# harskish/ganspace

Measured on NVIDIA H100. Metric: latent samples/sec into PCA (StyleGAN2-ffhq W, N=1e6), higher is better.
Workload: dtype f32

## Files before the change

### ganspace_b200/csrc/mapping_tc.cu

```cuda
#include "tc_common.cuh"
#include <stdlib.h>

namespace gsb {

constexpr int TC_BLOCK_M = 128;
constexpr int TC_BLOCK_N = 128;
constexpr int TC_BLOCK_K = 64;
constexpr int TC_STAGES = 3;
constexpr int TC_FRAG_ROWS = 64;
constexpr uint32_t TC_A_BYTES = TC_BLOCK_M * TC_BLOCK_K * 2;
constexpr uint32_t TC_W_BYTES = TC_BLOCK_N * TC_BLOCK_K * 2;
constexpr uint32_t TC_STAGE_BYTES = 2 * TC_A_BYTES + 2 * TC_W_BYTES;
constexpr uint32_t TC_BOX_BYTES = TC_FRAG_ROWS * 128;
constexpr uint32_t TC_STAGING_BYTES = 2 * 2 * TC_BOX_BYTES;
constexpr int TC_THREADS = tc::CONSUMER_THREADS + 128;
constexpr uint32_t TC_SMEM_BYTES = TC_STAGES * TC_STAGE_BYTES + TC_STAGING_BYTES + 64  + 1024 ;
static_assert(TC_SMEM_BYTES <= 232448, "mapping_layer_tc_kernel: shared memory exceeds the H100's 227 KB per block");

struct TcParams {
    const float *bias;
    __half *out_hi;
    __half *out_lo;
    float *out_f32;
    unsigned *overflow;
    const float *inv_wscale;
    int M, N_total, K;
    int mode;
    int dbg;
};

__global__ void __launch_bounds__(TC_THREADS, 1)
mapping_layer_tc_kernel(const __grid_constant__ CUtensorMap tm_a_hi, const __grid_constant__ CUtensorMap tm_a_lo,
                        const __grid_constant__ CUtensorMap tm_w_hi, const __grid_constant__ CUtensorMap tm_w_lo,
                        const __grid_constant__ CUtensorMap tm_o0, const __grid_constant__ CUtensorMap tm_o1,
                        const TcParams p) {
    using namespace tc;
    extern __shared__ uint8_t smem_raw[];
    uint8_t *smem = reinterpret_cast<uint8_t *>((reinterpret_cast<uintptr_t>(smem_raw) + 1023) & ~(uintptr_t)1023);
    uint8_t *staging = smem + TC_STAGES * TC_STAGE_BYTES;
    uint64_t *bars = reinterpret_cast<uint64_t *>(staging + TC_STAGING_BYTES);
    uint64_t *full_bar = bars;
    uint64_t *empty_bar = bars + TC_STAGES;
    uint64_t *turn_bar = bars + 2 * TC_STAGES;

    const int warp = threadIdx.x >> 5, lane = threadIdx.x & 31;
    const int num_m_tiles = (p.M + TC_BLOCK_M - 1) / TC_BLOCK_M;
    const int num_n_tiles = (p.N_total + TC_BLOCK_N - 1) / TC_BLOCK_N;
    const int num_k_blocks = (p.K + TC_BLOCK_K - 1) / TC_BLOCK_K;
    const int num_units = num_m_tiles * num_n_tiles;

    if (threadIdx.x == 0) {
        for (int s = 0; s < TC_STAGES; ++s) { mbar_init(&full_bar[s], 1); mbar_init(&empty_bar[s], 4); }
        mbar_init(&turn_bar[0], 4); mbar_init(&turn_bar[1], 4);
        mbar_fence_init();
    }
    if (warp == PRODUCER_WARP && lane == 0) {
        tma_prefetch_desc(&tm_a_hi); tma_prefetch_desc(&tm_a_lo);
        tma_prefetch_desc(&tm_w_hi); tma_prefetch_desc(&tm_w_lo);
        tma_prefetch_desc(&tm_o0); tma_prefetch_desc(&tm_o1);
    }
    __syncthreads();

    if (warp >= PRODUCER_WARP) {
        asm volatile("setmaxnreg.dec.sync.aligned.u32 40;");
        if (warp == PRODUCER_WARP && lane == 0) {
            int stage = 0; uint32_t phase = 0;
            for (int u = blockIdx.x; u < num_units; u += gridDim.x) {
                const int m0 = (u / num_n_tiles) * TC_BLOCK_M, n0 = (u % num_n_tiles) * TC_BLOCK_N;
                for (int kb = 0; kb < num_k_blocks; ++kb) {
                    mbar_wait(&empty_bar[stage], phase ^ 1);
                    uint8_t *st = smem + stage * TC_STAGE_BYTES;
                    mbar_arrive_expect_tx(&full_bar[stage], ((p.dbg & 4) ? 0u : 2 * TC_A_BYTES) + ((p.dbg & 2) ? 0u : 2 * TC_W_BYTES));
                    if (!(p.dbg & 4)) {
                        tma_load_2d(&tm_a_hi, &full_bar[stage], st, kb * TC_BLOCK_K, m0);
                        tma_load_2d(&tm_a_lo, &full_bar[stage], st + TC_A_BYTES, kb * TC_BLOCK_K, m0);
                    }
                    if (!(p.dbg & 2)) {
                        tma_load_2d(&tm_w_hi, &full_bar[stage], st + 2 * TC_A_BYTES, kb * TC_BLOCK_K, n0);
                        tma_load_2d(&tm_w_lo, &full_bar[stage], st + 2 * TC_A_BYTES + TC_W_BYTES, kb * TC_BLOCK_K, n0);
                    }
                    if (++stage == TC_STAGES) { stage = 0; phase ^= 1; }
                }
            }
        }
    } else {
        asm volatile("setmaxnreg.inc.sync.aligned.u32 232;");
        const int wg = warp >> 2;
        const int rr0 = (warp & 3) * 16 + (lane >> 2);
        const int q2 = 2 * (lane & 3);
        const bool has_bias = (p.mode != 1);
        const float slope = (p.mode == 0) ? 0.2f : 1.0f, gain = (p.mode == 0) ? 1.41421356237309515f : 1.0f;
        const float inv_wscale = __ldg(p.inv_wscale);
        uint8_t *stg = staging + wg * (2 * TC_BOX_BYTES);
        const bool storer = ((threadIdx.x & 127) == 0);
        const bool to_f32 = (p.out_f32 != nullptr);
        bool ovf = false;
        float acc0[64], acc1[64];
#pragma unroll
        for (int j = 0; j < 64; ++j) { acc0[j] = 0.f; acc1[j] = 0.f; }

        auto store_chunk = [&](const float (&acc)[64], const int ib, const int mrow, const int n0, const int c0) {
            if (storer) asm volatile("cp.async.bulk.wait_group.read 0;" ::: "memory");
            asm volatile("bar.sync %0, 128;" ::"r"(1 + wg) : "memory");
#pragma unroll
            for (int g = 0; g < 8; ++g) {
                const int col = n0 + c0 + 8 * g + q2;
                float2 b = make_float2(0.f, 0.f);
                if (has_bias && col < p.N_total) b = __ldg(reinterpret_cast<const float2 *>(p.bias + col));
#pragma unroll
                for (int h = 0; h < 2; ++h) {
                    const int rr = rr0 + 8 * h;
                    float f[2];
#pragma unroll
                    for (int e = 0; e < 2; ++e) {
                        float x = __fmul_rn(acc[ib + 4 * g + 2 * h + e], inv_wscale) + (e ? b.y : b.x);
                        x = (x >= 0.f) ? x : __fmul_rn(x, slope);
                        f[e] = __fmul_rn(gain, x);
                    }
                    uint8_t *row = stg + rr * 128;
                    const uint32_t sw = (uint32_t)(rr & 7);
                    if (to_f32) {
                        const int cb = (8 * g + q2) & 31;
                        *reinterpret_cast<float2 *>(row + (g >> 2) * TC_BOX_BYTES + ((((uint32_t)cb >> 2) ^ sw) << 4) + (cb & 3) * 4) =
                            make_float2(f[0], f[1]);
                    } else {
                        uint32_t hi, lo;
                        split2(f[0], f[1], hi, lo);
                        ovf |= (fabsf(f[0]) > 60000.f) | (fabsf(f[1]) > 60000.f);
                        *reinterpret_cast<uint32_t *>(row + (((uint32_t)g ^ sw) << 4) + 2 * q2) = hi;
                        *reinterpret_cast<uint32_t *>(row + TC_BOX_BYTES + (((uint32_t)g ^ sw) << 4) + 2 * q2) = lo;
                    }
                }
            }
            asm volatile("fence.proxy.async.shared::cta;" ::: "memory");
            asm volatile("bar.sync %0, 128;" ::"r"(1 + wg) : "memory");
            if (storer && !(p.dbg & 1) && n0 + c0 < p.N_total) {
                if (to_f32) {
                    tma_store_2d(&tm_o0, stg, n0 + c0, mrow);
                    if (n0 + c0 + 32 < p.N_total) tma_store_2d(&tm_o0, stg + TC_BOX_BYTES, n0 + c0 + 32, mrow);
                } else {
                    tma_store_2d(&tm_o0, stg, n0 + c0, mrow);
                    tma_store_2d(&tm_o1, stg + TC_BOX_BYTES, n0 + c0, mrow);
                }
                asm volatile("cp.async.bulk.commit_group;" ::: "memory");
            }
        };

        for (int i = wg;; i += 2) {
            const int u = blockIdx.x + i * gridDim.x;
            if (u >= num_units) break;
            const int m0 = (u / num_n_tiles) * TC_BLOCK_M, n0 = (u % num_n_tiles) * TC_BLOCK_N;
            const int g0 = i * num_k_blocks;
            int stage = g0 % TC_STAGES, prev = stage;
            uint32_t phase = (uint32_t)(g0 / TC_STAGES) & 1;
            if (i > 0) mbar_wait(&turn_bar[wg], (uint32_t)((i - 1) >> 1) & 1);
            for (int kb = 0; kb < num_k_blocks; ++kb) {
                mbar_wait(&full_bar[stage], phase);
                if (!(p.dbg & 8)) {
                    const uint32_t st = smem_u32(smem + stage * TC_STAGE_BYTES);
                    const uint32_t sw = st + 2 * TC_A_BYTES;
                    const uint64_t d_wh = sw128_kmajor_desc(sw), d_wl = sw128_kmajor_desc(sw + TC_W_BYTES);
                    wgmma_fence();
                    split_kblock_m64n128(acc0, sw128_kmajor_desc(st), sw128_kmajor_desc(st + TC_A_BYTES), d_wh, d_wl, kb > 0);
                    split_kblock_m64n128(acc1, sw128_kmajor_desc(st + TC_A_BYTES / 2),
                                         sw128_kmajor_desc(st + TC_A_BYTES + TC_A_BYTES / 2), d_wh, d_wl, kb > 0);
                    wgmma_commit();
                }
                wgmma_wait_1();
                if (kb > 0 && lane == 0) mbar_arrive(&empty_bar[prev]);
                if (kb == num_k_blocks - 1 && lane == 0) mbar_arrive(&turn_bar[wg ^ 1]);
                prev = stage;
                if (++stage == TC_STAGES) { stage = 0; phase ^= 1; }
            }
            wgmma_wait_all();
            if (lane == 0) mbar_arrive(&empty_bar[prev]);
            store_chunk(acc0, 0, m0, n0, 0);
            store_chunk(acc0, 32, m0, n0, 64);
            store_chunk(acc1, 0, m0 + TC_FRAG_ROWS, n0, 0);
            store_chunk(acc1, 32, m0 + TC_FRAG_ROWS, n0, 64);
        }
        if (ovf) atomicOr(p.overflow, 1u);
        if (storer) asm volatile("cp.async.bulk.wait_group 0;" ::: "memory");
    }
}

__global__ void pixelnorm_split_kernel(const float *__restrict__ x, __half *__restrict__ hi, __half *__restrict__ lo,
                                       int64_t n, int dim, int do_norm, unsigned *overflow) {
    int64_t row = blockIdx.x * (int64_t)(blockDim.x >> 5) + (threadIdx.x >> 5);
    if (row >= n) return;
    const int lane = threadIdx.x & 31;
    const float4 *xr = reinterpret_cast<const float4 *>(x + row * dim);
    float r = 1.f;
    if (do_norm) {
        float s = 0.f;
        for (int i = lane; i < dim / 4; i += 32) {
            float4 v = xr[i];
            s += v.x * v.x + v.y * v.y + v.z * v.z + v.w * v.w;
        }
        s = warp_sum(s);
        r = 1.0f / sqrtf(s / (float)dim + 1e-8f);
    }
    bool ovf = false;
    for (int i = lane; i < dim / 4; i += 32) {
        float4 v = xr[i];
        const float f[4] = {v.x * r, v.y * r, v.z * r, v.w * r};
        uint2 ph, pl;
        ovf |= tc::split4(f, ph, pl);
        reinterpret_cast<uint2 *>(hi + row * dim)[i] = ph;
        reinterpret_cast<uint2 *>(lo + row * dim)[i] = pl;
    }
    if (ovf) atomicOr(overflow, 1u);
}

__global__ void pick_wscale_kernel(const float *__restrict__ absmax, float *__restrict__ wscale,
                                   float *__restrict__ inv_wscale) {
    float m = *absmax;
    if (!(m > 0.f)) m = 1.f;
    int e = 0;
    frexpf(m, &e);
    const int s = 14 - e;
    *wscale = ldexpf(1.f, s);
    *inv_wscale = ldexpf(1.f, -s);
}

__global__ void weight_split_kernel(const float *__restrict__ pw, int64_t count, const float *__restrict__ wscale_p,
                                    __half *__restrict__ hi, __half *__restrict__ lo) {
    const float wscale = *wscale_p;
    for (int64_t i = blockIdx.x * (int64_t)blockDim.x + threadIdx.x; i < count; i += (int64_t)gridDim.x * blockDim.x) {
        tc::split1(pw[i] * wscale, hi[i], lo[i]);
    }
}

__global__ void absmax_kernel(const float *__restrict__ x, int64_t count, float *__restrict__ out) {
    float m = 0.f;
    for (int64_t i = blockIdx.x * (int64_t)blockDim.x + threadIdx.x; i < count; i += (int64_t)gridDim.x * blockDim.x)
        m = fmaxf(m, fabsf(x[i]));
    for (int o = 16; o > 0; o >>= 1) m = fmaxf(m, __shfl_xor_sync(0xffffffffu, m, o));
    if ((threadIdx.x & 31) == 0) atomicMax(reinterpret_cast<int *>(out), __float_as_int(m));
}

static int make_tmap(CUtensorMap *map, const void *base, uint64_t rows, uint64_t cols, uint32_t box_rows,
                     CUtensorMapDataType type = CU_TENSOR_MAP_DATA_TYPE_FLOAT16) {
    const uint32_t esize = (type == CU_TENSOR_MAP_DATA_TYPE_FLOAT32) ? 4 : 2;
    const uint64_t dims[2] = {cols, rows};
    const uint64_t strides[1] = {cols * esize};
    const uint32_t box[2] = {128 / esize, box_rows};
    return tc_make_tmap(map, type, base, 2, dims, strides, box);
}

size_t mapping_tc_packed_bytes(int n_layers, int dim) {
    return align_up((size_t)n_layers * dim * dim * 2, 256) * 2 + align_up((size_t)3 * n_layers * sizeof(float), 256) + 256;
}

struct TcPackView {
    __half *w_hi, *w_lo;
    float *inv_wscale, *wscale, *absmax;
    unsigned *overflow;
};
static TcPackView tc_pack_view(void *base, int n_layers, int dim) {
    TcPackView v;
    char *p = reinterpret_cast<char *>(base);
    size_t wb = align_up((size_t)n_layers * dim * dim * 2, 256);
    v.w_hi = reinterpret_cast<__half *>(p);
    v.w_lo = reinterpret_cast<__half *>(p + wb);
    v.inv_wscale = reinterpret_cast<float *>(p + 2 * wb);
    v.wscale = v.inv_wscale + n_layers;
    v.absmax = v.wscale + n_layers;
    v.overflow = reinterpret_cast<unsigned *>(p + 2 * wb + align_up((size_t)3 * n_layers * sizeof(float), 256));
    return v;
}

int mapping_tc_pack(const float *pw, int n_layers, int dim, void *tc_base, cudaStream_t st) {
    TcPackView v = tc_pack_view(tc_base, n_layers, dim);
    GSB_CHECK_CUDA(cudaMemsetAsync(v.inv_wscale, 0, (size_t)3 * n_layers * sizeof(float), st));
    GSB_CHECK_CUDA(cudaMemsetAsync(v.overflow, 0, sizeof(unsigned), st));
    const int64_t per = (int64_t)dim * dim;
    for (int l = 0; l < n_layers; ++l) {
        absmax_kernel<<<64, 256, 0, st>>>(pw + l * per, per, v.absmax + l);
        GSB_CHECK_LAUNCH();
        pick_wscale_kernel<<<1, 1, 0, st>>>(v.absmax + l, v.wscale + l, v.inv_wscale + l);
        GSB_CHECK_LAUNCH();
        weight_split_kernel<<<256, 256, 0, st>>>(pw + l * per, per, v.wscale + l, v.w_hi + l * per, v.w_lo + l * per);
        GSB_CHECK_LAUNCH();
    }
    return GSB_OK;
}

static int tc_ensure_attr() {
    static bool attr_set = false;
    if (!attr_set) {
        GSB_CHECK_CUDA(cudaFuncSetAttribute(mapping_layer_tc_kernel, cudaFuncAttributeMaxDynamicSharedMemorySize, (int)TC_SMEM_BYTES));
        attr_set = true;
    }
    return GSB_OK;
}

static int tc_launch_layer(const CUtensorMap &tm_ah, const CUtensorMap &tm_al, const CUtensorMap &tm_wh, const CUtensorMap &tm_wl,
                           TcParams p, int leave_free_sms, cudaStream_t st) {
    CUtensorMap tm_o0, tm_o1;
    if (p.out_f32) {
        if (int r = make_tmap(&tm_o0, p.out_f32, (uint64_t)p.M, (uint64_t)p.N_total, TC_FRAG_ROWS,
                              CU_TENSOR_MAP_DATA_TYPE_FLOAT32))
            return r;
        tm_o1 = tm_o0;
    } else {
        if (int r = make_tmap(&tm_o0, p.out_hi, (uint64_t)p.M, (uint64_t)p.N_total, TC_FRAG_ROWS)) return r;
        if (int r = make_tmap(&tm_o1, p.out_lo, (uint64_t)p.M, (uint64_t)p.N_total, TC_FRAG_ROWS)) return r;
    }
    const int m_tiles = (p.M + TC_BLOCK_M - 1) / TC_BLOCK_M, n_tiles = (p.N_total + TC_BLOCK_N - 1) / TC_BLOCK_N;
    int avail = num_sms() - leave_free_sms;
    if (avail < 16) avail = 16;
    if (avail > num_sms()) avail = num_sms();
    {
        static int dbg = -1;
        if (dbg < 0) { const char *e = getenv("GANSPACE_B200_MAPPING_DBG"); dbg = e ? atoi(e) : 0; }
        p.dbg = dbg;
    }
    const int64_t units = (int64_t)m_tiles * n_tiles;
    const int grid = units < avail ? (int)units : avail;
    mapping_layer_tc_kernel<<<grid, TC_THREADS, TC_SMEM_BYTES, st>>>(tm_ah, tm_al, tm_wh, tm_wl, tm_o0, tm_o1, p);
    GSB_CHECK_LAUNCH();
    return GSB_OK;
}

int tc_gemm_plain(const __half *a_hi, const __half *a_lo, int64_t M, int K, const __half *w_hi, const __half *w_lo, int N,
                  const float *inv_wscale, float *out, unsigned *overflow, int leave_free_sms, cudaStream_t st) {
    GSB_CHECK_ARG(N % 32 == 0 && N >= 32 && K % 8 == 0 && K >= 8 && M > 0 && M < (1ll << 31),
                  "tc_gemm_plain: need N%%32==0, K%%8==0 (M=%lld N=%d K=%d)", (long long)M, N, K);
    if (int r = tc_ensure_attr()) return r;
    CUtensorMap tm_ah, tm_al, tm_wh, tm_wl;
    if (int r = make_tmap(&tm_ah, a_hi, (uint64_t)M, (uint64_t)K, TC_BLOCK_M)) return r;
    if (int r = make_tmap(&tm_al, a_lo, (uint64_t)M, (uint64_t)K, TC_BLOCK_M)) return r;
    if (int r = make_tmap(&tm_wh, w_hi, (uint64_t)N, (uint64_t)K, TC_BLOCK_N)) return r;
    if (int r = make_tmap(&tm_wl, w_lo, (uint64_t)N, (uint64_t)K, TC_BLOCK_N)) return r;
    TcParams p;
    p.bias = nullptr; p.out_hi = nullptr; p.out_lo = nullptr; p.out_f32 = out; p.overflow = overflow;
    p.inv_wscale = inv_wscale; p.M = (int)M; p.N_total = N; p.K = K; p.mode = 1;
    return tc_launch_layer(tm_ah, tm_al, tm_wh, tm_wl, p, leave_free_sms, st);
}

size_t tc_linear_workspace_bytes(int64_t n, int N, int K) {
    return 2 * align_up((size_t)n * K * 2, 256) + 2 * align_up((size_t)N * K * 2, 256) + 512;
}

int tc_linear(const float *x, const float *w, const float *bias, float *y, int64_t n, int N, int K, bool lrelu, void *ws,
              cudaStream_t st) {
    GSB_CHECK_ARG(N % 256 == 0 && K % TC_BLOCK_K == 0 && n > 0 && n < (1ll << 31) && bias, "tc_linear: need N%%256==0, K%%64==0, bias");
    if (int r = tc_ensure_attr()) return r;
    char *p0 = reinterpret_cast<char *>(ws);
    const size_t xb = align_up((size_t)n * K * 2, 256), wb = align_up((size_t)N * K * 2, 256);
    __half *x_hi = (__half *)p0, *x_lo = (__half *)(p0 + xb), *w_hi = (__half *)(p0 + 2 * xb), *w_lo = (__half *)(p0 + 2 * xb + wb);
    float *scal = (float *)(p0 + 2 * xb + 2 * wb);
    unsigned *overflow = (unsigned *)(p0 + 2 * xb + 2 * wb + 256);
    GSB_CHECK_CUDA(cudaMemsetAsync(scal, 0, 512, st));
    absmax_kernel<<<256, 256, 0, st>>>(w, (int64_t)N * K, scal + 2);
    GSB_CHECK_LAUNCH();
    pick_wscale_kernel<<<1, 1, 0, st>>>(scal + 2, scal + 1, scal);
    GSB_CHECK_LAUNCH();
    weight_split_kernel<<<1024, 256, 0, st>>>(w, (int64_t)N * K, scal + 1, w_hi, w_lo);
    GSB_CHECK_LAUNCH();
    pixelnorm_split_kernel<<<(unsigned)((n + 7) / 8), 256, 0, st>>>(x, x_hi, x_lo, n, K, 0, overflow);
    GSB_CHECK_LAUNCH();
    CUtensorMap tm_ah, tm_al, tm_wh, tm_wl;
    if (int r = make_tmap(&tm_ah, x_hi, (uint64_t)n, (uint64_t)K, TC_BLOCK_M)) return r;
    if (int r = make_tmap(&tm_al, x_lo, (uint64_t)n, (uint64_t)K, TC_BLOCK_M)) return r;
    if (int r = make_tmap(&tm_wh, w_hi, (uint64_t)N, (uint64_t)K, TC_BLOCK_N)) return r;
    if (int r = make_tmap(&tm_wl, w_lo, (uint64_t)N, (uint64_t)K, TC_BLOCK_N)) return r;
    TcParams p;
    p.bias = bias; p.out_hi = nullptr; p.out_lo = nullptr; p.out_f32 = y; p.overflow = overflow;
    p.inv_wscale = scal; p.M = (int)n; p.N_total = N; p.K = K; p.mode = lrelu ? 0 : 2;
    return tc_launch_layer(tm_ah, tm_al, tm_wh, tm_wl, p, 0, st);
}

int mapping_forward_tc(const float *pb, void *tc_base, int n_layers, int dim,
                       const float *d_z, float *d_w, int64_t n, bool pixelnorm, void *ws, int leave_free_sms,
                       cudaStream_t st) {
    GSB_CHECK_ARG(dim % 256 == 0 && dim % TC_BLOCK_K == 0, "mapping_forward_tc: dim must be a multiple of 256");
    GSB_CHECK_ARG(n < (1ll << 31), "mapping_forward_tc: too many rows");
    TcPackView v = tc_pack_view(tc_base, n_layers, dim);
    const size_t buf = align_up((size_t)n * dim * 2, 256);
    __half *a_hi[2] = {reinterpret_cast<__half *>(ws), reinterpret_cast<__half *>((char *)ws + 2 * buf)};
    __half *a_lo[2] = {reinterpret_cast<__half *>((char *)ws + buf), reinterpret_cast<__half *>((char *)ws + 3 * buf)};

    if (int r = tc_ensure_attr()) return r;
    pixelnorm_split_kernel<<<(unsigned)((n + 7) / 8), 256, 0, st>>>(d_z, a_hi[0], a_lo[0], n, dim, pixelnorm ? 1 : 0,
                                                                  v.overflow);
    GSB_CHECK_LAUNCH();
    const int64_t per = (int64_t)dim * dim;
    for (int l = 0; l < n_layers; ++l) {
        const int src = l & 1, dst = src ^ 1;
        CUtensorMap tm_ah, tm_al, tm_wh, tm_wl;
        if (int r = make_tmap(&tm_ah, a_hi[src], (uint64_t)n, dim, TC_BLOCK_M)) return r;
        if (int r = make_tmap(&tm_al, a_lo[src], (uint64_t)n, dim, TC_BLOCK_M)) return r;
        if (int r = make_tmap(&tm_wh, v.w_hi + l * per, dim, dim, TC_BLOCK_N)) return r;
        if (int r = make_tmap(&tm_wl, v.w_lo + l * per, dim, dim, TC_BLOCK_N)) return r;
        TcParams p;
        p.bias = pb + (int64_t)l * dim;
        const bool last = (l == n_layers - 1);
        p.out_hi = last ? nullptr : a_hi[dst];
        p.out_lo = last ? nullptr : a_lo[dst];
        p.out_f32 = last ? d_w : nullptr;
        p.overflow = v.overflow;
        p.inv_wscale = v.inv_wscale + l;
        p.M = (int)n; p.N_total = dim; p.K = dim; p.mode = 0;
        if (int r = tc_launch_layer(tm_ah, tm_al, tm_wh, tm_wl, p, leave_free_sms, st)) return r;
    }
    return GSB_OK;
}

size_t mapping_tc_workspace_bytes(int64_t n, int dim) { return 4 * align_up((size_t)n * dim * 2, 256); }

unsigned *mapping_tc_overflow_flag(void *tc_base, int n_layers, int dim) {
    return tc_pack_view(tc_base, n_layers, dim).overflow;
}

}
```

### ganspace_b200/csrc/synthesis.cu

```cuda
#include "tc_common.cuh"
#include <math.h>

namespace gsb {

constexpr int SY_MAX_LAYERS = 24;
constexpr int SY_CHUNK_ROWS = 2048;

struct SynthLayerView {
    __half *w_hi, *w_lo;
    float *scal;
    float *wsq;
    float *modw;
    float *modb;
    float *actb;
    float *noise;
};
struct SynthView {
    float *const_nhwc;
    float *zeros;
    unsigned *overflow;
    SynthLayerView L[SY_MAX_LAYERS];
    size_t bytes;
};
static int res_out_of(const gsb_styled_conv &l) { return l.upsample ? 2 * l.res_in : l.res_in; }
// ... 163 lines not shown
    for (int k = 0; k < 4; ++k) f[k] = sqrt2 * ((f[k] >= 0.f) ? f[k] : 0.2f * f[k]);
    if (e.rgb_w) {
        const float4 sr = *reinterpret_cast<const float4 *>(e.rgb_s + b * c + 4 * q);
        const float g[4] = {f[0] * sr.x, f[1] * sr.y, f[2] * sr.z, f[3] * sr.w};
        float r[3];
#pragma unroll
        for (int o = 0; o < 3; ++o) {
            const float4 wv = *reinterpret_cast<const float4 *>(e.rgb_w + (int64_t)o * c + 4 * q);
            r[o] = e.rgb_scale * (g[0] * wv.x + g[1] * wv.y + g[2] * wv.z + g[3] * wv.w);
        }
        const int cq = c >> 2, span = cq < 32 ? cq : 32;
        for (int off = span >> 1; off > 0; off >>= 1) {
#pragma unroll
            for (int o = 0; o < 3; ++o) r[o] += __shfl_xor_sync(0xffffffffu, r[o], off);
        }
        float *dst = e.rgb_out + (b * hw + pix) * 3;
        if (cq <= 32) {
            if ((q & (span - 1)) == 0) { dst[0] += r[0]; dst[1] += r[1]; dst[2] += r[2]; }
        } else {
            __shared__ float rgb_red[8][3];
            const int wib = threadIdx.x >> 5, wpp = cq >> 5;
            if ((threadIdx.x & 31) == 0) { rgb_red[wib][0] = r[0]; rgb_red[wib][1] = r[1]; rgb_red[wib][2] = r[2]; }
            __syncthreads();
            if ((threadIdx.x & 31) == 0 && (wib % wpp) == 0) {
                float t0 = 0.f, t1 = 0.f, t2 = 0.f;
                for (int k = 0; k < wpp; ++k) { t0 += rgb_red[wib + k][0]; t1 += rgb_red[wib + k][1]; t2 += rgb_red[wib + k][2]; }
                dst[0] += t0; dst[1] += t1; dst[2] += t2;
            }
            __syncthreads();
        }
    }
    if (e.s_next) {
        const float4 sn = *reinterpret_cast<const float4 *>(e.s_next + b * c + 4 * q);
        f[0] *= sn.x; f[1] *= sn.y; f[2] *= sn.z; f[3] *= sn.w;
        bool ovf = false;
        store_split4(f, e.out_hi, e.out_lo, (b * hw + pix) * (int64_t)c + 4 * q, ovf);
        if (ovf) atomicOr(e.overflow, 1u);
    } else if (e.out_f32) {
        *reinterpret_cast<float4 *>(e.out_f32 + b * e.ld + (int64_t)pix * c + 4 * q) = make_float4(f[0], f[1], f[2], f[3]);
    }
}

__global__ void sy_rgb_init_kernel(const float *__restrict__ bias, const float *__restrict__ prev, int64_t n, int R, float *__restrict__ rgb) {
    const int64_t idx = blockIdx.x * (int64_t)blockDim.x + threadIdx.x;
    if (idx >= n * R * R) return;
    const int x = (int)(idx % R), y = (int)((idx / R) % R);
    const int64_t b = idx / ((int64_t)R * R);
    float acc[3] = {bias[0], bias[1], bias[2]};
    if (prev) {
        const int Rp = R >> 1;
        const float k1[4] = {1.f, 3.f, 3.f, 1.f};
#pragma unroll
        for (int i = 0; i < 4; ++i) {
            const int u = y + i - 2;
            if (u < 0 || (u & 1) || (u >> 1) >= Rp) continue;
#pragma unroll
            for (int j = 0; j < 4; ++j) {
                const int v = x + j - 2;
                if (v < 0 || (v & 1) || (v >> 1) >= Rp) continue;
                const float kw = k1[i] * k1[j] * 0.0625f;
                const float *pp = prev + ((b * Rp + (u >> 1)) * Rp + (v >> 1)) * 3;
                acc[0] = fmaf(kw, pp[0], acc[0]); acc[1] = fmaf(kw, pp[1], acc[1]); acc[2] = fmaf(kw, pp[2], acc[2]);
            }
        }
    }
    float *o = rgb + idx * 3;
    o[0] = acc[0]; o[1] = acc[1]; o[2] = acc[2];
}

__global__ void __launch_bounds__(256)
sy_conv_gather_kernel(const float *__restrict__ Y, int64_t nb, int H, int W, int c, EpiParams e) {
    const int cq = c >> 2;
    const int64_t idx = blockIdx.x * (int64_t)blockDim.x + threadIdx.x;
    if (idx >= nb * H * W * cq) return;
    const int q = (int)(idx % cq);
    const int64_t pixg = idx / cq;
    const int x = (int)(pixg % W), y = (int)((pixg / W) % H);
    const int64_t b = pixg / ((int64_t)W * H);
    float4 acc = make_float4(0.f, 0.f, 0.f, 0.f);
#pragma unroll
    for (int ky = 0; ky < 3; ++ky) {
        const int yy = y + ky - 1;
        if (yy < 0 || yy >= H) continue;
#pragma unroll
        for (int kx = 0; kx < 3; ++kx) {
            const int xx = x + kx - 1;
            if (xx < 0 || xx >= W) continue;
            const float4 v = *reinterpret_cast<const float4 *>(Y + ((b * H + yy) * W + xx) * (int64_t)(9 * c) + (ky * 3 + kx) * c + 4 * q);
            acc.x += v.x; acc.y += v.y; acc.z += v.z; acc.w += v.w;
        }
    }
    sy_epilogue(e, acc, b, y * W + x, H * W, c, q);
}

__global__ void __launch_bounds__(256)
sy_upconv_scatter_kernel(const float *__restrict__ Y, int64_t nb, int H, int W, int c, float *__restrict__ T) {
    const int cq = c >> 2, TH = 2 * H + 1, TW = 2 * W + 1;
    const int64_t idx = blockIdx.x * (int64_t)blockDim.x + threadIdx.x;
    if (idx >= nb * TH * TW * cq) return;
    const int q = (int)(idx % cq);
    const int64_t pixg = idx / cq;
    const int v = (int)(pixg % TW), u = (int)((pixg / TW) % TH);
    const int64_t b = pixg / ((int64_t)TW * TH);
    float4 acc = make_float4(0.f, 0.f, 0.f, 0.f);
#pragma unroll
    for (int ky = 0; ky < 3; ++ky) {
        const int t = u - ky;
        if (t < 0 || (t & 1) || (t >> 1) >= H) continue;
        const int yy = t >> 1;
#pragma unroll
        for (int kx = 0; kx < 3; ++kx) {
            const int s = v - kx;
            if (s < 0 || (s & 1) || (s >> 1) >= W) continue;
            const int xx = s >> 1;
            const float4 w = *reinterpret_cast<const float4 *>(Y + ((b * H + yy) * W + xx) * (int64_t)(9 * c) + (ky * 3 + kx) * c + 4 * q);
            acc.x += w.x; acc.y += w.y; acc.z += w.z; acc.w += w.w;
        }
    }
    *reinterpret_cast<float4 *>(T + pixg * c + 4 * q) = acc;
}

__global__ void __launch_bounds__(256)
sy_blur_epilogue_kernel(const float *__restrict__ T, int64_t nb, int H2, int W2, int c, EpiParams e) {
    const int cq = c >> 2, TH = H2 + 1, TW = W2 + 1;
    const int64_t idx = blockIdx.x * (int64_t)blockDim.x + threadIdx.x;
    if (idx >= nb * H2 * W2 * cq) return;
    const int q = (int)(idx % cq);
    const int64_t pixg = idx / cq;
    const int x = (int)(pixg % W2), y = (int)((pixg / W2) % H2);
    const int64_t b = pixg / ((int64_t)W2 * H2);
    const float k1[4] = {1.f, 3.f, 3.f, 1.f};
    float4 acc = make_float4(0.f, 0.f, 0.f, 0.f);
#pragma unroll
    for (int i = 0; i < 4; ++i) {
        const int u = y + i - 1;
        if (u < 0 || u >= TH) continue;
#pragma unroll
        for (int j = 0; j < 4; ++j) {
            const int v = x + j - 1;
            if (v < 0 || v >= TW) continue;
            const float kw = k1[i] * k1[j] * 0.0625f;
            const float4 t = *reinterpret_cast<const float4 *>(T + ((b * TH + u) * TW + v) * (int64_t)c + 4 * q);
            acc.x = fmaf(kw, t.x, acc.x); acc.y = fmaf(kw, t.y, acc.y); acc.z = fmaf(kw, t.z, acc.z); acc.w = fmaf(kw, t.w, acc.w);
        }
    }
    sy_epilogue(e, acc, b, y * W2 + x, H2 * W2, c, q);
}

struct SynthWs {
    float *S[SY_MAX_LAYERS], *D[SY_MAX_LAYERS];
    float *s2;
    __half *act[2][2];
    float *Y, *T;
    float *rgb[2], *rgb_s, *rgb_modw;
    size_t bytes;
};
static int chunk_samples(const gsb_styled_conv &c) {
    int spc = SY_CHUNK_ROWS / (c.res_in * c.res_in);
    return spc < 1 ? 1 : spc;
}
static SynthWs synth_ws(void *base, const gsb_styled_conv *layers, int n_run, int64_t n, bool with_rgb = false, int style_dim = 0) {
    SynthWs w;
    char *p = reinterpret_cast<char *>(base);
    size_t off = 0;
    auto take = [&](size_t bytes) { char *q = p + off; off += align_up(bytes, 256); return q; };
    size_t cmax = 0, act_elems = 0, y_elems = 0, t_elems = 0;
    for (int l = 0; l < n_run; ++l) {
        const gsb_styled_conv &c = layers[l];
        w.S[l] = (float *)take((size_t)n * c.cin * 4);
        w.D[l] = (float *)take((size_t)n * c.cout * 4);
        cmax = cmax > (size_t)c.cin ? cmax : (size_t)c.cin;
        const size_t in_elems = (size_t)n * c.res_in * c.res_in * c.cin;
        act_elems = act_elems > in_elems ? act_elems : in_elems;
        const size_t spc = (size_t)chunk_samples(c);
        const size_t ye = spc * c.res_in * c.res_in * 9 * c.cout;
        y_elems = y_elems > ye ? y_elems : ye;
        if (c.upsample) {
            const size_t te = spc * (2 * c.res_in + 1) * (2 * c.res_in + 1) * c.cout;
            t_elems = t_elems > te ? t_elems : te;
        }
    }
    w.s2 = (float *)take((size_t)n * cmax * 4);
    for (int a = 0; a < 2; ++a)
        for (int h = 0; h < 2; ++h) w.act[a][h] = (__half *)take(act_elems * 2);
    w.Y = (float *)take(y_elems * 4);
    w.T = (float *)take((t_elems ? t_elems : 64) * 4);
    w.rgb[0] = w.rgb[1] = w.rgb_s = w.rgb_modw = nullptr;
    if (with_rgb) {
        const int ro = res_out_of(layers[n_run - 1]);
        size_t cm = 0;
        for (int l = 0; l < n_run; ++l) cm = cm > (size_t)layers[l].cout ? cm : (size_t)layers[l].cout;
        for (int a = 0; a < 2; ++a) w.rgb[a] = (float *)take((size_t)n * ro * ro * 3 * 4);
        w.rgb_s = (float *)take((size_t)n * cm * 4);
        w.rgb_modw = (float *)take(cm * (size_t)style_dim * 4);
    }
    w.bytes = off;
    return w;
}

}

extern "C" size_t gsb_synthesis_packed_bytes(const gsb_styled_conv *layers, int n_layers, int style_dim) {
    if (gsb::check_layers(layers, n_layers, style_dim)) return 0;
    return gsb::synth_view(nullptr, layers, n_layers, style_dim).bytes;
}

extern "C" int gsb_synthesis_pack(const gsb_styled_conv *layers, int n_layers, int style_dim, const float *d_const_input,
                                  void *d_packed, size_t packed_bytes, gsb_stream_t stream) {
    using namespace gsb;
    if (int r = check_layers(layers, n_layers, style_dim)) return r;
    GSB_CHECK_ARG(d_const_input && d_packed, "synthesis_pack: null pointer");
    SynthView v = synth_view(d_packed, layers, n_layers, style_dim);
    if (packed_bytes < v.bytes) { set_error("synthesis_pack: buffer too small (%zu < %zu)", packed_bytes, v.bytes); return GSB_ERR_WORKSPACE; }
    cudaStream_t st = (cudaStream_t)stream;
    GSB_CHECK_CUDA(cudaMemsetAsync(d_packed, 0, v.bytes, st));
    const int c0 = layers[0].cin;
    sy_const_nhwc_kernel<<<(16 * c0 + 255) / 256, 256, 0, st>>>(d_const_input, c0, v.const_nhwc);
    GSB_CHECK_LAUNCH();
    for (int l = 0; l < n_layers; ++l) {
        const gsb_styled_conv &c = layers[l];
        GSB_CHECK_ARG(c.conv_weight && c.mod_weight && c.mod_bias && c.act_bias && c.noise && c.noise_weight,
                      "synthesis_pack: layer %d has a null parameter pointer", l);
        const float scale = (float)(1.0 / sqrt((double)c.cin * 9.0));
        const float mscale = (float)(1.0 / sqrt((double)style_dim));
        const int64_t wcount = (int64_t)c.cout * c.cin * 9;
        sy_absmax_kernel<<<128, 256, 0, st>>>(c.conv_weight, wcount, scale, v.L[l].scal + 2);
        GSB_CHECK_LAUNCH();
        sy_pick_scale_kernel<<<1, 1, 0, st>>>(v.L[l].scal);
        GSB_CHECK_LAUNCH();
        sy_weight_pack_kernel<<<256, 256, 0, st>>>(c.conv_weight, c.cout, c.cin, scale, v.L[l].scal, v.L[l].w_hi, v.L[l].w_lo, v.L[l].wsq);
        GSB_CHECK_LAUNCH();
        sy_scale_copy_kernel<<<128, 256, 0, st>>>(c.mod_weight, (int64_t)c.cin * style_dim, mscale, nullptr, v.L[l].modw);
        GSB_CHECK_LAUNCH();
        sy_scale_copy_kernel<<<4, 256, 0, st>>>(c.mod_bias, c.cin, 1.0f, nullptr, v.L[l].modb);
        GSB_CHECK_LAUNCH();
        sy_scale_copy_kernel<<<4, 256, 0, st>>>(c.act_bias, c.cout, 1.0f, nullptr, v.L[l].actb);
        GSB_CHECK_LAUNCH();
        const int ro = res_out_of(c);
        sy_scale_copy_kernel<<<64, 256, 0, st>>>(c.noise, (int64_t)ro * ro, 1.0f, c.noise_weight, v.L[l].noise);
        GSB_CHECK_LAUNCH();
    }
    return GSB_OK;
}

extern "C" size_t gsb_synthesis_workspace_bytes(const gsb_styled_conv *layers, int n_run, int64_t n) {
    if (!layers || n_run < 1 || n_run > gsb::SY_MAX_LAYERS || n < 1) return 0;
    return gsb::synth_ws(nullptr, layers, n_run, n).bytes;
}

namespace gsb {

static int synthesis_run(const void *d_packed, const gsb_styled_conv *layers, int n_layers, int n_run, int style_dim,
                         const gsb_to_rgb *rgbs, int n_rgb, const float *d_w, int w_layers, int64_t n, float *d_out, int64_t ld_out,
                         float *d_rgb_out, void *d_workspace, size_t workspace_bytes, gsb_stream_t stream) {
    if (int r = check_layers(layers, n_layers, style_dim)) return r;
    GSB_CHECK_ARG(d_packed && d_w && d_workspace && (d_out || d_rgb_out), "synthesis: null pointer");
    GSB_CHECK_ARG(n_run >= 1 && n_run <= n_layers && w_layers >= 1, "synthesis: n_run / w_layers out of range");
    GSB_CHECK_ARG(n_rgb >= 0 && (n_rgb == 0 || (rgbs && d_rgb_out && 2 * (n_rgb - 1) <= n_run - 1)), "synthesis: bad ToRGB list");
    if (n == 0) return GSB_OK;
    const gsb_styled_conv &last = layers[n_run - 1];
    const int ro_last = res_out_of(last);
    GSB_CHECK_ARG(n > 0 && (!d_out || (ld_out >= (int64_t)ro_last * ro_last * last.cout && ld_out % 4 == 0)), "synthesis: bad n / ld_out");
    SynthView v = synth_view(const_cast<void *>(d_packed), layers, n_layers, style_dim);
    SynthWs w = synth_ws(d_workspace, layers, n_run, n, n_rgb > 0, style_dim);
    if (workspace_bytes < w.bytes) { set_error("synthesis: workspace too small (%zu < %zu)", workspace_bytes, w.bytes); return GSB_ERR_WORKSPACE; }
    cudaStream_t st = (cudaStream_t)stream;
    auto latent = [&](int idx) { return d_w + (size_t)(idx < w_layers ? idx : w_layers - 1) * n * style_dim; };

    for (int l = 0; l < n_run; ++l) {
        const gsb_styled_conv &c = layers[l];
        if (int r = sy_linear(latent(l), v.L[l].modw, v.L[l].modb, w.S[l], n, c.cin, style_dim, stream)) return r;
        const int64_t cnt = n * c.cin;
        sy_square_kernel<<<(unsigned)((cnt + 255) / 256), 256, 0, st>>>(w.S[l], cnt, w.s2);
        GSB_CHECK_LAUNCH();
        if (int r = sy_linear(w.s2, v.L[l].wsq, v.zeros, w.D[l], n, c.cout, c.cin, stream)) return r;
        const int64_t cnt2 = n * c.cout;
        sy_rsqrt_eps_kernel<<<(unsigned)((cnt2 + 255) / 256), 256, 0, st>>>(w.D[l], cnt2);
        GSB_CHECK_LAUNCH();
    }
    {
        const int64_t total = n * 16 * (layers[0].cin / 4);
        sy_const_modulate_kernel<<<(unsigned)((total + 255) / 256), 256, 0, st>>>(v.const_nhwc, w.S[0], n, 16, layers[0].cin, w.act[0][0],
                                                                                w.act[0][1], v.overflow);
        GSB_CHECK_LAUNCH();
    }
    const float *rgb_prev = nullptr;
    for (int l = 0; l < n_run; ++l) {
        const gsb_styled_conv &c = layers[l];
        const int src = l & 1, dst = src ^ 1;
        const bool hooked = (l == n_run - 1);
        const int H = c.res_in, ro = res_out_of(c), hw_in = H * H, hw_out = ro * ro;
        const int spc = chunk_samples(c);
        const int j = l / 2;
        const bool with_rgb = (l % 2 == 0) && j < n_rgb;
        float *rgb_cur = nullptr;
        if (with_rgb) {
            const gsb_to_rgb &t = rgbs[j];
            GSB_CHECK_ARG(t.conv_weight && t.mod_weight && t.mod_bias && t.bias && t.cin == c.cout && (c.cout & (c.cout - 1)) == 0,
                          "synthesis: ToRGB %d does not match layer %d (cin=%d, cout=%d)", j, l, t.cin, c.cout);
            rgb_cur = (j == n_rgb - 1) ? d_rgb_out : w.rgb[j & 1];
            const float mscale = (float)(1.0 / sqrt((double)style_dim));
            sy_scale_copy_kernel<<<64, 256, 0, st>>>(t.mod_weight, (int64_t)c.cout * style_dim, mscale, nullptr, w.rgb_modw);
            GSB_CHECK_LAUNCH();
            if (int r = sy_linear(latent(2 * j + 1), w.rgb_modw, t.mod_bias, w.rgb_s, n, c.cout, style_dim, stream)) return r;
            const int64_t tot = n * hw_out;
            sy_rgb_init_kernel<<<(unsigned)((tot + 255) / 256), 256, 0, st>>>(t.bias, rgb_prev, n, ro, rgb_cur);
            GSB_CHECK_LAUNCH();
        }
        for (int64_t b0 = 0; b0 < n; b0 += spc) {
            const int64_t nb = (b0 + spc <= n) ? spc : (n - b0);
            const int64_t rows = nb * hw_in;
            if (int r = tc_gemm_plain(w.act[src][0] + b0 * hw_in * c.cin, w.act[src][1] + b0 * hw_in * c.cin, rows, c.cin, v.L[l].w_hi,
                                      v.L[l].w_lo, 9 * c.cout, v.L[l].scal, w.Y, v.overflow, 0, st)) return r;
            EpiParams e;
            e.demod = w.D[l] + b0 * c.cout;
            e.noise = v.L[l].noise;
            e.bias = v.L[l].actb;
            e.s_next = hooked ? nullptr : w.S[l + 1] + b0 * c.cout;
            e.out_hi = hooked ? nullptr : w.act[dst][0] + b0 * hw_out * c.cout;
            e.out_lo = hooked ? nullptr : w.act[dst][1] + b0 * hw_out * c.cout;
            e.out_f32 = (hooked && d_out) ? d_out + b0 * ld_out : nullptr;
            e.ld = ld_out;
            e.overflow = v.overflow;
            e.rgb_w = with_rgb ? rgbs[j].conv_weight : nullptr;
            e.rgb_s = with_rgb ? w.rgb_s + b0 * c.cout : nullptr;
            e.rgb_out = with_rgb ? rgb_cur + b0 * hw_out * 3 : nullptr;
            e.rgb_scale = (float)(1.0 / sqrt((double)c.cout));
            const int cq = c.cout / 4;
            if (c.upsample) {
                const int64_t t_total = nb * (2 * H + 1) * (2 * H + 1) * cq;
                sy_upconv_scatter_kernel<<<(unsigned)((t_total + 255) / 256), 256, 0, st>>>(w.Y, nb, H, H, c.cout, w.T);
                GSB_CHECK_LAUNCH();
                const int64_t o_total = nb * hw_out * cq;
                sy_blur_epilogue_kernel<<<(unsigned)((o_total + 255) / 256), 256, 0, st>>>(w.T, nb, ro, ro, c.cout, e);
                GSB_CHECK_LAUNCH();
            } else {
                const int64_t o_total = nb * hw_out * cq;
                sy_conv_gather_kernel<<<(unsigned)((o_total + 255) / 256), 256, 0, st>>>(w.Y, nb, H, H, c.cout, e);
                GSB_CHECK_LAUNCH();
            }
        }
        if (with_rgb) rgb_prev = rgb_cur;
    }
    return GSB_OK;
}

}

extern "C" int gsb_synthesis_forward(const void *d_packed, const gsb_styled_conv *layers, int n_layers, int n_run, int style_dim,
                                     const float *d_w, int64_t n, float *d_out, int64_t ld_out, void *d_workspace,
                                     size_t workspace_bytes, gsb_stream_t stream) {
    GSB_CHECK_ARG(d_out, "synthesis_forward: null output");
    return gsb::synthesis_run(d_packed, layers, n_layers, n_run, style_dim, nullptr, 0, d_w, 1, n, d_out, ld_out, nullptr, d_workspace,
                              workspace_bytes, stream);
}

extern "C" size_t gsb_synthesis_render_workspace_bytes(const gsb_styled_conv *layers, int n_run, int64_t n, int style_dim) {
    if (!layers || n_run < 1 || n_run > gsb::SY_MAX_LAYERS || n < 1) return 0;
    return gsb::synth_ws(nullptr, layers, n_run, n, true, style_dim).bytes;
}

extern "C" int gsb_synthesis_render(const void *d_packed, const gsb_styled_conv *layers, int n_layers, int n_run, int style_dim,
                                    const gsb_to_rgb *rgbs, int n_rgb, const float *d_w, int w_layers, int64_t n, float *d_act_out,
                                    int64_t ld_act, float *d_rgb_out, void *d_workspace, size_t workspace_bytes, gsb_stream_t stream) {
    return gsb::synthesis_run(d_packed, layers, n_layers, n_run, style_dim, rgbs, n_rgb, d_w, w_layers, n, d_act_out, ld_act, d_rgb_out,
                              d_workspace, workspace_bytes, stream);
}

extern "C" int gsb_synthesis_status(const void *d_packed, const gsb_styled_conv *layers, int n_layers, int style_dim, unsigned *h_flags) {
    using namespace gsb;
    if (int r = check_layers(layers, n_layers, style_dim)) return r;
    GSB_CHECK_ARG(d_packed && h_flags, "synthesis_status: null pointer");
    SynthView v = synth_view(const_cast<void *>(d_packed), layers, n_layers, style_dim);
    GSB_CHECK_CUDA(cudaMemcpy(h_flags, v.overflow, sizeof(unsigned), cudaMemcpyDeviceToHost));
    return GSB_OK;
}
```

### ganspace_b200/csrc/tc_common.cuh

```cuda
#pragma once
#include "common.cuh"
#include <cuda.h>
#include <cuda_fp16.h>

namespace gsb {
namespace tc {

constexpr int CONSUMER_THREADS = 256;
constexpr int THREADS = CONSUMER_THREADS + 32;
constexpr int PRODUCER_WARP = CONSUMER_THREADS / 32;

__device__ __forceinline__ uint32_t smem_u32(const void *p) { return (uint32_t)__cvta_generic_to_shared(p); }

__device__ __forceinline__ void mbar_init(uint64_t *bar, uint32_t count) {
    asm volatile("mbarrier.init.shared::cta.b64 [%0], %1;" ::"r"(smem_u32(bar)), "r"(count));
}
__device__ __forceinline__ void mbar_fence_init() { asm volatile("fence.mbarrier_init.release.cluster;" ::: "memory"); }
__device__ __forceinline__ void mbar_wait(uint64_t *bar, uint32_t parity) {
    asm volatile(
        "{\n\t"
        ".reg .pred P1;\n\t"
        "TCW_LOOP:\n\t"
        "mbarrier.try_wait.parity.shared::cta.b64 P1, [%0], %1, 0x989680;\n\t"
        "@P1 bra TCW_DONE;\n\t"
        "bra TCW_LOOP;\n\t"
        "TCW_DONE:\n\t"
        "}" ::"r"(smem_u32(bar)), "r"(parity)
        : "memory");
}
__device__ __forceinline__ void mbar_arrive(uint64_t *bar) {
    asm volatile("mbarrier.arrive.shared::cta.b64 _, [%0];" ::"r"(smem_u32(bar)) : "memory");
}
__device__ __forceinline__ void mbar_arrive_expect_tx(uint64_t *bar, uint32_t bytes) {
    asm volatile("mbarrier.arrive.expect_tx.shared::cta.b64 _, [%0], %1;" ::"r"(smem_u32(bar)), "r"(bytes) : "memory");
}

__device__ __forceinline__ void tma_prefetch_desc(const CUtensorMap *map) {
    asm volatile("prefetch.tensormap [%0];" ::"l"(map) : "memory");
}
__device__ __forceinline__ void tma_load_2d(const CUtensorMap *map, uint64_t *bar, void *dst, int c0, int c1) {
    asm volatile(
        "cp.async.bulk.tensor.2d.shared::cluster.global.mbarrier::complete_tx::bytes [%0], [%1, {%3, %4}], [%2];"
        ::"r"(smem_u32(dst)), "l"(map), "r"(smem_u32(bar)), "r"(c0), "r"(c1)
        : "memory");
}
__device__ __forceinline__ void tma_load_3d(const CUtensorMap *map, uint64_t *bar, void *dst, int c0, int c1, int c2) {
    asm volatile(
        "cp.async.bulk.tensor.3d.shared::cluster.global.mbarrier::complete_tx::bytes [%0], [%1, {%3, %4, %5}], [%2];"
        ::"r"(smem_u32(dst)), "l"(map), "r"(smem_u32(bar)), "r"(c0), "r"(c1), "r"(c2)
        : "memory");
}
__device__ __forceinline__ void tma_store_2d(const CUtensorMap *map, const void *src, int c0, int c1) {
    asm volatile("cp.async.bulk.tensor.2d.global.shared::cta.bulk_group [%0, {%2, %3}], [%1];"
                 ::"l"(map), "r"(smem_u32(src)), "r"(c0), "r"(c1) : "memory");
}

__device__ __forceinline__ void wgmma_fence() { asm volatile("wgmma.fence.sync.aligned;" ::: "memory"); }
__device__ __forceinline__ void wgmma_commit() { asm volatile("wgmma.commit_group.sync.aligned;" ::: "memory"); }
__device__ __forceinline__ void wgmma_wait_all() { asm volatile("wgmma.wait_group.sync.aligned 0;" ::: "memory"); }
__device__ __forceinline__ void wgmma_wait_1() { asm volatile("wgmma.wait_group.sync.aligned 1;" ::: "memory"); }

__device__ __forceinline__ uint64_t sw128_kmajor_desc(uint32_t smem_addr) {
    uint64_t d = 0;
    d |= (uint64_t)((smem_addr & 0x3FFFF) >> 4);
    d |= (uint64_t)1 << 16;
    d |= (uint64_t)(1024 >> 4) << 32;
    d |= (uint64_t)1 << 62;
    return d;
}

__device__ __forceinline__ void wgmma_m64n128(float (&d)[64], uint64_t da, uint64_t db, uint32_t accumulate) {
    asm volatile(
        "{\n\t"
        ".reg .pred p;\n\t"
        "setp.ne.b32 p, %66, 0;\n\t"
        "wgmma.mma_async.sync.aligned.m64n128k16.f32.f16.f16 "
        "{%0, %1, %2, %3, %4, %5, %6, %7, %8, %9, %10, %11, %12, %13, %14, %15, "
        "%16, %17, %18, %19, %20, %21, %22, %23, %24, %25, %26, %27, %28, %29, %30, %31, "
        "%32, %33, %34, %35, %36, %37, %38, %39, %40, %41, %42, %43, %44, %45, %46, %47, "
        "%48, %49, %50, %51, %52, %53, %54, %55, %56, %57, %58, %59, %60, %61, %62, %63}, "
        "%64, %65, p, 1, 1, 0, 0;\n\t"
        "}"
        : "+f"(d[0]), "+f"(d[1]), "+f"(d[2]), "+f"(d[3]), "+f"(d[4]), "+f"(d[5]), "+f"(d[6]), "+f"(d[7]),
          "+f"(d[8]), "+f"(d[9]), "+f"(d[10]), "+f"(d[11]), "+f"(d[12]), "+f"(d[13]), "+f"(d[14]), "+f"(d[15]),
          "+f"(d[16]), "+f"(d[17]), "+f"(d[18]), "+f"(d[19]), "+f"(d[20]), "+f"(d[21]), "+f"(d[22]), "+f"(d[23]),
          "+f"(d[24]), "+f"(d[25]), "+f"(d[26]), "+f"(d[27]), "+f"(d[28]), "+f"(d[29]), "+f"(d[30]), "+f"(d[31]),
          "+f"(d[32]), "+f"(d[33]), "+f"(d[34]), "+f"(d[35]), "+f"(d[36]), "+f"(d[37]), "+f"(d[38]), "+f"(d[39]),
          "+f"(d[40]), "+f"(d[41]), "+f"(d[42]), "+f"(d[43]), "+f"(d[44]), "+f"(d[45]), "+f"(d[46]), "+f"(d[47]),
          "+f"(d[48]), "+f"(d[49]), "+f"(d[50]), "+f"(d[51]), "+f"(d[52]), "+f"(d[53]), "+f"(d[54]), "+f"(d[55]),
          "+f"(d[56]), "+f"(d[57]), "+f"(d[58]), "+f"(d[59]), "+f"(d[60]), "+f"(d[61]), "+f"(d[62]), "+f"(d[63])
        : "l"(da), "l"(db), "r"(accumulate)
        : "memory");
}

__device__ __forceinline__ void split_kblock_m64n128(float (&d)[64], uint64_t ah, uint64_t al, uint64_t bh, uint64_t bl,
                                                     bool accumulate) {
#pragma unroll
    for (int k = 0; k < 4; ++k) {
        const uint64_t koff = (uint64_t)(2 * k);
        wgmma_m64n128(d, ah + koff, bh + koff, (accumulate || k > 0) ? 1u : 0u);
        wgmma_m64n128(d, al + koff, bh + koff, 1u);
        wgmma_m64n128(d, ah + koff, bl + koff, 1u);
    }
}

__device__ __forceinline__ void split1(float x, __half &hi, __half &lo) {
    hi = __float2half_rn(x);
    lo = __float2half_rn(x - __half2float(hi));
}
__device__ __forceinline__ void split2(float a, float b, uint32_t &hi, uint32_t &lo) {
    __half h0, h1, l0, l1;
    split1(a, h0, l0);
    split1(b, h1, l1);
    hi = (uint32_t)__half_as_ushort(h0) | ((uint32_t)__half_as_ushort(h1) << 16);
    lo = (uint32_t)__half_as_ushort(l0) | ((uint32_t)__half_as_ushort(l1) << 16);
}
__device__ __forceinline__ bool split4(const float (&f)[4], uint2 &hi, uint2 &lo) {
    split2(f[0], f[1], hi.x, lo.x);
    split2(f[2], f[3], hi.y, lo.y);
    return (fabsf(f[0]) > 60000.f) | (fabsf(f[1]) > 60000.f) | (fabsf(f[2]) > 60000.f) | (fabsf(f[3]) > 60000.f);
}

}

int tc_make_tmap(CUtensorMap *map, CUtensorMapDataType type, const void *base, int rank, const uint64_t *dims,
                 const uint64_t *strides_bytes, const uint32_t *box);

enum class GramEpilogue { Store, Accumulate };
int gram_tc_launch(GramEpilogue epi, const __half *hi, const __half *lo, int64_t k, int64_t k_pitch, int n_groups, int n_pad,
                   int n_rows, const int *exps, double *out, cudaStream_t st);
size_t gram_tc_workspace_bytes(int n_pad, int64_t d);
bool gram_tc_supported(int64_t d);
int gram_tc(const float *M, int n_rows, int n_pad, int64_t d, void *ws, double *T, cudaStream_t st);

bool stats_tc_supported(int64_t nb, int d);
size_t stats_tc_workspace_bytes(int n_groups, int64_t nb, int d);
int stats_tc(const float *x, int n_groups, int64_t nb, int d, int64_t ld, double *mean, double *gram, void *ws, cudaStream_t st);

size_t mapping_tc_packed_bytes(int n_layers, int dim);
int mapping_tc_pack(const float *pw, int n_layers, int dim, void *tc_base, cudaStream_t st);
int mapping_forward_tc(const float *pb, void *tc_base, int n_layers, int dim, const float *d_z, float *d_w,
                       int64_t n, bool pixelnorm, void *ws, int leave_free_sms, cudaStream_t st);
size_t mapping_tc_workspace_bytes(int64_t n, int dim);
unsigned *mapping_tc_overflow_flag(void *tc_base, int n_layers, int dim);
size_t tc_linear_workspace_bytes(int64_t n, int N, int K);
int tc_linear(const float *x, const float *w, const float *bias, float *y, int64_t n, int N, int K, bool lrelu, void *ws,
              cudaStream_t st);
int tc_gemm_plain(const __half *a_hi, const __half *a_lo, int64_t M, int K, const __half *w_hi, const __half *w_lo, int N,
                  const float *inv_wscale, float *out, unsigned *overflow, int leave_free_sms, cudaStream_t st);

}
```

Baseline: 17.77 million.

## Replace static tile striding with atomic work-queue tile scheduler in mapping TC kernel

The persistent mapping-layer GEMM kernel now pulls tiles from a global atomic counter instead of a fixed blockIdx stride. The producer warp claims the next tile during the last k-block of the current one and hands it to the alternating consumer warpgroups through new tile_full/tile_empty mbarriers and a shared slot. The aim is to balance load across SMs when tile counts don't divide evenly and some SMs run slower. In exchange it adds an atomic per tile, a memset per launch, and extra barrier handshakes between producer and consumers.

Measured after the change: 19.17 million (median of 6 runs). +7.9%, better.

```diff
diff --git a/ganspace_b200/csrc/mapping_tc.cu b/ganspace_b200/csrc/mapping_tc.cu
--- a/ganspace_b200/csrc/mapping_tc.cu
+++ b/ganspace_b200/csrc/mapping_tc.cu
@@ -14,7 +14,7 @@
 constexpr uint32_t TC_BOX_BYTES = TC_FRAG_ROWS * 128;
 constexpr uint32_t TC_STAGING_BYTES = 2 * 2 * TC_BOX_BYTES;
 constexpr int TC_THREADS = tc::CONSUMER_THREADS + 128;
-constexpr uint32_t TC_SMEM_BYTES = TC_STAGES * TC_STAGE_BYTES + TC_STAGING_BYTES + 64  + 1024 ;
+constexpr uint32_t TC_SMEM_BYTES = TC_STAGES * TC_STAGE_BYTES + TC_STAGING_BYTES + 128  + 1024 ;
 static_assert(TC_SMEM_BYTES <= 232448, "mapping_layer_tc_kernel: shared memory exceeds the H100's 227 KB per block");
 
 struct TcParams {
@@ -23,6 +23,7 @@
     __half *out_lo;
     float *out_f32;
     unsigned *overflow;
+    unsigned *queue;
     const float *inv_wscale;
     int M, N_total, K;
     int mode;
@@ -42,6 +43,9 @@
     uint64_t *full_bar = bars;
     uint64_t *empty_bar = bars + TC_STAGES;
     uint64_t *turn_bar = bars + 2 * TC_STAGES;
+    uint64_t *tile_full = bars + 2 * TC_STAGES + 2;
+    uint64_t *tile_empty = bars + 2 * TC_STAGES + 4;
+    volatile int *tile_slot = reinterpret_cast<volatile int *>(bars + 2 * TC_STAGES + 6);
 
     const int warp = threadIdx.x >> 5, lane = threadIdx.x & 31;
     const int num_m_tiles = (p.M + TC_BLOCK_M - 1) / TC_BLOCK_M;
@@ -51,7 +55,7 @@
 
     if (threadIdx.x == 0) {
         for (int s = 0; s < TC_STAGES; ++s) { mbar_init(&full_bar[s], 1); mbar_init(&empty_bar[s], 4); }
-        mbar_init(&turn_bar[0], 4); mbar_init(&turn_bar[1], 4);
+        for (int w = 0; w < 2; ++w) { mbar_init(&turn_bar[w], 4); mbar_init(&tile_full[w], 1); mbar_init(&tile_empty[w], 4); }
         mbar_fence_init();
     }
     if (warp == PRODUCER_WARP && lane == 0) {
@@ -65,9 +69,23 @@
         asm volatile("setmaxnreg.dec.sync.aligned.u32 40;");
         if (warp == PRODUCER_WARP && lane == 0) {
             int stage = 0; uint32_t phase = 0;
-            for (int u = blockIdx.x; u < num_units; u += gridDim.x) {
+            int u = (int)atomicAdd(p.queue, 1u);
+            for (int i = 0;; ++i) {
+                const int wg = i & 1;
+                mbar_wait(&tile_empty[wg], ((uint32_t)(i >> 1) & 1) ^ 1);
+                if (u >= num_units) {
+                    tile_slot[wg] = -1;
+                    mbar_arrive(&tile_full[wg]);
+                    mbar_wait(&tile_empty[wg ^ 1], ((uint32_t)((i + 1) >> 1) & 1) ^ 1);
+                    tile_slot[wg ^ 1] = -1;
+                    mbar_arrive(&tile_full[wg ^ 1]);
+                    break;
+                }
+                tile_slot[wg] = u;
+                mbar_arrive(&tile_full[wg]);
                 const int m0 = (u / num_n_tiles) * TC_BLOCK_M, n0 = (u % num_n_tiles) * TC_BLOCK_N;
                 for (int kb = 0; kb < num_k_blocks; ++kb) {
+                    if (kb == num_k_blocks - 1) u = (int)atomicAdd(p.queue, 1u);
                     mbar_wait(&empty_bar[stage], phase ^ 1);
                     uint8_t *st = smem + stage * TC_STAGE_BYTES;
                     mbar_arrive_expect_tx(&full_bar[stage], ((p.dbg & 4) ? 0u : 2 * TC_A_BYTES) + ((p.dbg & 2) ? 0u : 2 * TC_W_BYTES));
@@ -147,8 +165,11 @@
         };
 
         for (int i = wg;; i += 2) {
-            const int u = blockIdx.x + i * gridDim.x;
-            if (u >= num_units) break;
+            mbar_wait(&tile_full[wg], (uint32_t)(i >> 1) & 1);
+            const int u = tile_slot[wg];
+            __syncwarp();
+            if (lane == 0) mbar_arrive(&tile_empty[wg]);
+            if (u < 0) break;
             const int m0 = (u / num_n_tiles) * TC_BLOCK_M, n0 = (u % num_n_tiles) * TC_BLOCK_N;
             const int g0 = i * num_k_blocks;
             int stage = g0 % TC_STAGES, prev = stage;
@@ -296,7 +317,7 @@
 }
 
 static int tc_launch_layer(const CUtensorMap &tm_ah, const CUtensorMap &tm_al, const CUtensorMap &tm_wh, const CUtensorMap &tm_wl,
-                           TcParams p, int leave_free_sms, cudaStream_t st) {
+                           TcParams p, unsigned *queue, int leave_free_sms, cudaStream_t st) {
     CUtensorMap tm_o0, tm_o1;
     if (p.out_f32) {
         if (int r = make_tmap(&tm_o0, p.out_f32, (uint64_t)p.M, (uint64_t)p.N_total, TC_FRAG_ROWS,
@@ -317,6 +338,9 @@
         p.dbg = dbg;
     }
     const int64_t units = (int64_t)m_tiles * n_tiles;
+    GSB_CHECK_ARG(units < (1ll << 31) - 1024, "mapping_layer_tc: too many tiles");
+    GSB_CHECK_CUDA(cudaMemsetAsync(queue, 0, sizeof(unsigned), st));
+    p.queue = queue;
     const int grid = units < avail ? (int)units : avail;
     mapping_layer_tc_kernel<<<grid, TC_THREADS, TC_SMEM_BYTES, st>>>(tm_ah, tm_al, tm_wh, tm_wl, tm_o0, tm_o1, p);
     GSB_CHECK_LAUNCH();
@@ -324,8 +348,8 @@
 }
 
 int tc_gemm_plain(const __half *a_hi, const __half *a_lo, int64_t M, int K, const __half *w_hi, const __half *w_lo, int N,
-                  const float *inv_wscale, float *out, unsigned *overflow, int leave_free_sms, cudaStream_t st) {
-    GSB_CHECK_ARG(N % 32 == 0 && N >= 32 && K % 8 == 0 && K >= 8 && M > 0 && M < (1ll << 31),
+                  const float *inv_wscale, float *out, unsigned *overflow, unsigned *queue, int leave_free_sms, cudaStream_t st) {
+    GSB_CHECK_ARG(N % 32 == 0 && N >= 32 && K % 8 == 0 && K >= 8 && M > 0 && M < (1ll << 31) && queue,
                   "tc_gemm_plain: need N%%32==0, K%%8==0 (M=%lld N=%d K=%d)", (long long)M, N, K);
     if (int r = tc_ensure_attr()) return r;
     CUtensorMap tm_ah, tm_al, tm_wh, tm_wl;
@@ -336,7 +360,7 @@
     TcParams p;
     p.bias = nullptr; p.out_hi = nullptr; p.out_lo = nullptr; p.out_f32 = out; p.overflow = overflow;
     p.inv_wscale = inv_wscale; p.M = (int)M; p.N_total = N; p.K = K; p.mode = 1;
-    return tc_launch_layer(tm_ah, tm_al, tm_wh, tm_wl, p, leave_free_sms, st);
+    return tc_launch_layer(tm_ah, tm_al, tm_wh, tm_wl, p, queue, leave_free_sms, st);
 }
 
 size_t tc_linear_workspace_bytes(int64_t n, int N, int K) {
@@ -369,7 +393,7 @@
     TcParams p;
     p.bias = bias; p.out_hi = nullptr; p.out_lo = nullptr; p.out_f32 = y; p.overflow = overflow;
     p.inv_wscale = scal; p.M = (int)n; p.N_total = N; p.K = K; p.mode = lrelu ? 0 : 2;
-    return tc_launch_layer(tm_ah, tm_al, tm_wh, tm_wl, p, 0, st);
+    return tc_launch_layer(tm_ah, tm_al, tm_wh, tm_wl, p, overflow + 1, 0, st);
 }
 
 int mapping_forward_tc(const float *pb, void *tc_base, int n_layers, int dim,
@@ -381,6 +405,7 @@
     const size_t buf = align_up((size_t)n * dim * 2, 256);
     __half *a_hi[2] = {reinterpret_cast<__half *>(ws), reinterpret_cast<__half *>((char *)ws + 2 * buf)};
     __half *a_lo[2] = {reinterpret_cast<__half *>((char *)ws + buf), reinterpret_cast<__half *>((char *)ws + 3 * buf)};
+    unsigned *queue = reinterpret_cast<unsigned *>((char *)ws + 4 * buf);
 
     if (int r = tc_ensure_attr()) return r;
     pixelnorm_split_kernel<<<(unsigned)((n + 7) / 8), 256, 0, st>>>(d_z, a_hi[0], a_lo[0], n, dim, pixelnorm ? 1 : 0,
@@ -403,12 +428,12 @@
         p.overflow = v.overflow;
         p.inv_wscale = v.inv_wscale + l;
         p.M = (int)n; p.N_total = dim; p.K = dim; p.mode = 0;
-        if (int r = tc_launch_layer(tm_ah, tm_al, tm_wh, tm_wl, p, leave_free_sms, st)) return r;
+        if (int r = tc_launch_layer(tm_ah, tm_al, tm_wh, tm_wl, p, queue, leave_free_sms, st)) return r;
     }
     return GSB_OK;
 }
 
-size_t mapping_tc_workspace_bytes(int64_t n, int dim) { return 4 * align_up((size_t)n * dim * 2, 256); }
+size_t mapping_tc_workspace_bytes(int64_t n, int dim) { return 4 * align_up((size_t)n * dim * 2, 256) + 256; }
 
 unsigned *mapping_tc_overflow_flag(void *tc_base, int n_layers, int dim) {
     return tc_pack_view(tc_base, n_layers, dim).overflow;
diff --git a/ganspace_b200/csrc/synthesis.cu b/ganspace_b200/csrc/synthesis.cu
--- a/ganspace_b200/csrc/synthesis.cu
+++ b/ganspace_b200/csrc/synthesis.cu
@@ -339,6 +339,7 @@
     float *s2;
     __half *act[2][2];
     float *Y, *T;
+    unsigned *queue;
     float *rgb[2], *rgb_s, *rgb_modw;
     size_t bytes;
 };
@@ -372,6 +373,7 @@
         for (int h = 0; h < 2; ++h) w.act[a][h] = (__half *)take(act_elems * 2);
     w.Y = (float *)take(y_elems * 4);
     w.T = (float *)take((t_elems ? t_elems : 64) * 4);
+    w.queue = (unsigned *)take(sizeof(unsigned));
     w.rgb[0] = w.rgb[1] = w.rgb_s = w.rgb_modw = nullptr;
     if (with_rgb) {
         const int ro = res_out_of(layers[n_run - 1]);
@@ -498,7 +500,7 @@
             const int64_t nb = (b0 + spc <= n) ? spc : (n - b0);
             const int64_t rows = nb * hw_in;
             if (int r = tc_gemm_plain(w.act[src][0] + b0 * hw_in * c.cin, w.act[src][1] + b0 * hw_in * c.cin, rows, c.cin, v.L[l].w_hi,
-                                      v.L[l].w_lo, 9 * c.cout, v.L[l].scal, w.Y, v.overflow, 0, st)) return r;
+                                      v.L[l].w_lo, 9 * c.cout, v.L[l].scal, w.Y, v.overflow, w.queue, 0, st)) return r;
             EpiParams e;
             e.demod = w.D[l] + b0 * c.cout;
             e.noise = v.L[l].noise;
diff --git a/ganspace_b200/csrc/tc_common.cuh b/ganspace_b200/csrc/tc_common.cuh
--- a/ganspace_b200/csrc/tc_common.cuh
+++ b/ganspace_b200/csrc/tc_common.cuh
@@ -147,6 +147,6 @@
 int tc_linear(const float *x, const float *w, const float *bias, float *y, int64_t n, int N, int K, bool lrelu, void *ws,
               cudaStream_t st);
 int tc_gemm_plain(const __half *a_hi, const __half *a_lo, int64_t M, int K, const __half *w_hi, const __half *w_lo, int N,
-                  const float *inv_wscale, float *out, unsigned *overflow, int leave_free_sms, cudaStream_t st);
+                  const float *inv_wscale, float *out, unsigned *overflow, unsigned *queue, int leave_free_sms, cudaStream_t st);
 
 }
```
